# nianticlabs/mickey

Hardware: NVIDIA H100
Metric: image-pairs/sec @720x540 (higher is better)
Workload: dtype f16 operands / f32 accumulate (tensor core), f32 matcher+solver

## Files before the change

mickey_b200/csrc/attention_tc.cu:

```cuda
#include "gemm_tc.cuh"
#include "ops.h"
#include "gemm.h"
#include <algorithm>
#include <cstdlib>
#include <cstring>

namespace mk {

constexpr int FA_BQ = 192, FA_BK = 128, FA_D = 64, FA_KV_STAGES = 4;
constexpr int FA_CONSUMERS = 3, FA_THREADS = 128 * (FA_CONSUMERS + 1), FA_WARP_TMA = 4 * FA_CONSUMERS;
constexpr int FA_REGS_PRODUCER = 32, FA_REGS_CONSUMER = 160;
static_assert(FA_REGS_PRODUCER * 128 + FA_REGS_CONSUMER * 128 * FA_CONSUMERS <= 65536, "attention: register budget");
constexpr int FA_Q_BYTES = FA_BQ * 128;
constexpr int FA_KV_BYTES = FA_BK * 128;
constexpr int FA_O_BYTES = 64 * 128;
constexpr int FA_REGION = 2 * FA_Q_BYTES + 2 * FA_KV_STAGES * FA_KV_BYTES + FA_CONSUMERS * FA_O_BYTES;
constexpr int FA_SMEM = FA_REGION + 1024 + 256;
static_assert(FA_SMEM <= 227 * 1024, "attention: shared memory");

__device__ __forceinline__ float ex2_approx(float x) {
  float y;
  asm("ex2.approx.ftz.f32 %0, %1;" : "=f"(y) : "f"(x));
  return y;
}

__device__ __forceinline__ void wgmma_m64n64k16_rs_tb(float (&d)[32], const uint32_t (&a)[4], uint64_t desc_b) {
  asm volatile(
      "{\n\t.reg .pred p;\n\tsetp.ne.b32 p, %37, 0;\n\t"
      "wgmma.mma_async.sync.aligned.m64n64k16.f32.f16.f16 "
      "{%0, %1, %2, %3, %4, %5, %6, %7, %8, %9, %10, %11, %12, %13, %14, %15, %16, %17, %18, %19, %20, %21, %22, %23, %24, %25, %26, %27, %28, %29, %30, %31}, {%32, %33, %34, %35}, %36, p, 1, 1, 1;\n\t}"
      : "+f"(d[0]), "+f"(d[1]), "+f"(d[2]), "+f"(d[3]), "+f"(d[4]), "+f"(d[5]), "+f"(d[6]), "+f"(d[7]), "+f"(d[8]), "+f"(d[9]), "+f"(d[10]), "+f"(d[11]), "+f"(d[12]), "+f"(d[13]), "+f"(d[14]), "+f"(d[15]), "+f"(d[16]), "+f"(d[17]), "+f"(d[18]), "+f"(d[19]), "+f"(d[20]), "+f"(d[21]), "+f"(d[22]), "+f"(d[23]), "+f"(d[24]), "+f"(d[25]), "+f"(d[26]), "+f"(d[27]), "+f"(d[28]), "+f"(d[29]), "+f"(d[30]), "+f"(d[31])
      : "r"(a[0]), "r"(a[1]), "r"(a[2]), "r"(a[3]), "l"(desc_b), "r"(1u));
}

__device__ __forceinline__ void warpgroup_sync(int wg) { asm volatile("bar.sync %0, 128;" ::"r"(2 + wg) : "memory"); }

struct AttnTile { int qt, head, im; };
__device__ __forceinline__ AttnTile attn_tile(int t, int q_tiles, int heads) {
  const int bh = t / q_tiles;
  return {t - bh * q_tiles, bh % heads, bh / heads};
}

__device__ __forceinline__ void softmax_tile(float (&s)[64], uint32_t (&p)[8][4], float (&m_run)[2], float (&l_run)[2],
                                             float (&alpha)[2], float scale_log2, int valid, int lane) {
  if (valid < FA_BK) {
#pragma unroll
    for (int i = 0; i < 64; ++i) {
      const int col = 8 * (i >> 2) + 2 * (lane & 3) + (i & 1);
      if (col >= valid) s[i] = -INFINITY;
    }
  }
#pragma unroll
  for (int h = 0; h < 2; ++h) {
    float mx = -INFINITY;
#pragma unroll
    for (int c = 0; c < 16; ++c) mx = fmaxf(mx, fmaxf(s[4 * c + 2 * h], s[4 * c + 2 * h + 1]));
    mx = fmaxf(mx, __shfl_xor_sync(0xffffffffu, mx, 1));
    mx = fmaxf(mx, __shfl_xor_sync(0xffffffffu, mx, 2));
    const float m_new = fmaxf(m_run[h], mx * scale_log2);
    alpha[h] = ex2_approx(m_run[h] - m_new);
    m_run[h] = m_new;
    float sum = 0.f;
#pragma unroll
    for (int c = 0; c < 16; ++c) {
      const float p0 = ex2_approx(fmaf(s[4 * c + 2 * h], scale_log2, -m_new));
      const float p1 = ex2_approx(fmaf(s[4 * c + 2 * h + 1], scale_log2, -m_new));
      const __half2 ph = __floats2half2_rn(p0, p1);
      const float2 r = __half22float2(ph);
      p[c >> 1][2 * (c & 1) + h] = *reinterpret_cast<const uint32_t*>(&ph);
      sum += r.x + r.y;
    }
    l_run[h] = l_run[h] * alpha[h] + sum;
  }
}

__global__ void __launch_bounds__(FA_THREADS, 1)
attention_tc_kernel(const __grid_constant__ CUtensorMap tmQ, const __grid_constant__ CUtensorMap tmKV,
                    const __grid_constant__ CUtensorMap tmO, int T, int heads, int q_tiles, int n_tiles_total, float scale_log2) {
  extern __shared__ uint8_t smem_raw[];
  const uint32_t raw = smem_u32(smem_raw);
  const uint32_t base = (raw + 1023u) & ~1023u;
  const uint32_t sQ = base;
  const uint32_t sK = sQ + 2 * FA_Q_BYTES;
  const uint32_t sV = sK + FA_KV_STAGES * FA_KV_BYTES;
  const uint32_t sO = sV + FA_KV_STAGES * FA_KV_BYTES;
  const uint32_t bars = base + FA_REGION;
  const uint32_t k_full = bars, k_empty = k_full + 8 * FA_KV_STAGES, v_full = k_empty + 8 * FA_KV_STAGES,
                 v_empty = v_full + 8 * FA_KV_STAGES, q_full = v_empty + 8 * FA_KV_STAGES, q_empty = q_full + 16;

  const int warp = threadIdx.x >> 5, lane = threadIdx.x & 31;
  const int D = heads * FA_D;
  const int n_kv = (T + FA_BK - 1) / FA_BK;

  if (warp == FA_WARP_TMA && lane == 0) {
    asm volatile("prefetch.tensormap [%0];" ::"l"(&tmQ) : "memory");
    asm volatile("prefetch.tensormap [%0];" ::"l"(&tmKV) : "memory");
    asm volatile("prefetch.tensormap [%0];" ::"l"(&tmO) : "memory");
    for (int s = 0; s < FA_KV_STAGES; ++s) {
      mbar_init(k_full + 8 * s, 1); mbar_init(k_empty + 8 * s, 4 * FA_CONSUMERS);
      mbar_init(v_full + 8 * s, 1); mbar_init(v_empty + 8 * s, 4 * FA_CONSUMERS);
    }
    for (int b = 0; b < 2; ++b) { mbar_init(q_full + 8 * b, 1); mbar_init(q_empty + 8 * b, 4 * FA_CONSUMERS); }
    asm volatile("fence.mbarrier_init.release.cluster;" ::: "memory");
  }
  __syncthreads();
  pdl_wait();

  if (warp >= FA_WARP_TMA) {
    setmaxnreg_dec<FA_REGS_PRODUCER>();
    if (warp == FA_WARP_TMA && elect_one()) {
      int st = 0;
      uint32_t ph = 0;
      int it = 0;
      for (int t = blockIdx.x; t < n_tiles_total; t += gridDim.x, ++it) {
        const AttnTile tile = attn_tile(t, q_tiles, heads);
        const int row_base = tile.im * T;
        const int qb = it & 1;
        mbar_wait(q_empty + 8 * qb, ((it >> 1) & 1) ^ 1);
        mbar_expect_tx(q_full + 8 * qb, FA_Q_BYTES);
        tma_load_2d(sQ + qb * FA_Q_BYTES, &tmQ, q_full + 8 * qb, tile.head * FA_D, row_base + tile.qt * FA_BQ);
        for (int j = 0; j < n_kv; ++j) {
          mbar_wait(k_empty + 8 * st, ph ^ 1);
          mbar_expect_tx(k_full + 8 * st, FA_KV_BYTES);
          tma_load_2d(sK + st * FA_KV_BYTES, &tmKV, k_full + 8 * st, D + tile.head * FA_D, row_base + j * FA_BK);
          mbar_wait(v_empty + 8 * st, ph ^ 1);
          mbar_expect_tx(v_full + 8 * st, FA_KV_BYTES);
          tma_load_2d(sV + st * FA_KV_BYTES, &tmKV, v_full + 8 * st, 2 * D + tile.head * FA_D, row_base + j * FA_BK);
          if (++st == FA_KV_STAGES) { st = 0; ph ^= 1; }
        }
      }
    }
    __syncwarp();
    pdl_trigger();
    return;
  }

  setmaxnreg_inc<FA_REGS_CONSUMER>();
  const int wg = warp >> 2;
  const uint32_t stage_o = sO + wg * FA_O_BYTES;
  int ks = 0, vs = 0;
  uint32_t kph = 0, vph = 0;
  int it = 0;
  for (int t = blockIdx.x; t < n_tiles_total; t += gridDim.x, ++it) {
    const AttnTile tile = attn_tile(t, q_tiles, heads);
    const int qb = it & 1;
    const uint64_t dq = gmma_desc_sw128(sQ + qb * FA_Q_BYTES + wg * (64 * 128));
    float s[64], o[32];
    uint32_t p[8][4];
#pragma unroll
    for (int i = 0; i < 32; ++i) o[i] = 0.f;
    float m_run[2] = {-INFINITY, -INFINITY}, l_run[2] = {0.f, 0.f}, alpha[2];
    mbar_wait(q_full + 8 * qb, (it >> 1) & 1);

    for (int j = 0; j < n_kv; ++j) {
      mbar_wait(k_full + 8 * ks, kph);
      const uint64_t dk = gmma_desc_sw128(sK + ks * FA_KV_BYTES);
      wgmma_fence();
#pragma unroll
      for (int k = 0; k < FA_D / WGMMA_K; ++k) wgmma_m64n128k16(s, dq + (uint64_t)(k * 2), dk + (uint64_t)(k * 2), k > 0 ? 1u : 0u);
      wgmma_commit();
      wgmma_wait<0>();
      reg_fence(s);
      if (lane == 0) mbar_arrive(k_empty + 8 * ks);
      if (++ks == FA_KV_STAGES) { ks = 0; kph ^= 1; }
      softmax_tile(s, p, m_run, l_run, alpha, scale_log2, T - j * FA_BK, lane);
#pragma unroll
      for (int c = 0; c < 8; ++c) {
        o[4 * c] *= alpha[0]; o[4 * c + 1] *= alpha[0];
        o[4 * c + 2] *= alpha[1]; o[4 * c + 3] *= alpha[1];
      }
      mbar_wait(v_full + 8 * vs, vph);
      const uint64_t dv = gmma_desc_sw128(sV + vs * FA_KV_BYTES);
      wgmma_fence();
#pragma unroll
      for (int kk = 0; kk < FA_BK / WGMMA_K; ++kk)
        wgmma_m64n64k16_rs_tb(o, p[kk], dv + (uint64_t)(kk * 128));
      wgmma_commit();
      wgmma_wait<0>();
      reg_fence(o);
      if (lane == 0) mbar_arrive(v_empty + 8 * vs);
      if (++vs == FA_KV_STAGES) { vs = 0; vph ^= 1; }
    }
    if (lane == 0) mbar_arrive(q_empty + 8 * qb);
    if (t + (int)gridDim.x >= n_tiles_total) pdl_trigger();

    const int row0 = tile.qt * FA_BQ + wg * 64;
    if (row0 >= T) continue;
    if (threadIdx.x % 128 == 0) tma_store_wait_read();
    warpgroup_sync(wg);
#pragma unroll
    for (int h = 0; h < 2; ++h) {
      float l = l_run[h];
      l += __shfl_xor_sync(0xffffffffu, l, 1);
      l += __shfl_xor_sync(0xffffffffu, l, 2);
      const float inv = 1.0f / l;
      const int r = (warp & 3) * 16 + (lane >> 2) + 8 * h;
#pragma unroll
      for (int c = 0; c < 8; ++c) {
        const __half2 v = __floats2half2_rn(o[4 * c + 2 * h] * inv, o[4 * c + 2 * h + 1] * inv);
        asm volatile("st.shared.b32 [%0], %1;" ::"r"(stage_o + r * 128 + ((c ^ (r & 7)) << 4) + 4 * (lane & 3)),
                     "r"(*reinterpret_cast<const uint32_t*>(&v)) : "memory");
      }
    }
    fence_async_smem();
    warpgroup_sync(wg);
    if (threadIdx.x % 128 == 0) {
      tma_store_3d(&tmO, stage_o, tile.head * FA_D, row0, tile.im);
      tma_store_commit();
    }
  }
  if (threadIdx.x % 128 == 0) tma_store_wait_all();
}

int attention_tc(const void* qkv, void* out, int n_img, int T, int D, int heads, cudaStream_t s) {
  if (D != heads * FA_D) { set_last_error("attention: head_dim must be 64 (D=%d heads=%d)", D, heads); return MK_ERR_UNSUPPORTED; }
  static unsigned long long attr_mask = 0;
  if (first_use_on_device(attr_mask)) {
    MK_CUDA_CHECK(cudaFuncSetAttribute(attention_tc_kernel, cudaFuncAttributeMaxDynamicSharedMemorySize, FA_SMEM));
  }
  CUtensorMap tmQ, tmKV, tmO;
  int rc = make_tensor_map_f16(&tmQ, qkv, (long long)n_img * T, 3LL * D, 3LL * D, FA_BQ);
  if (!rc) rc = make_tensor_map_f16(&tmKV, qkv, (long long)n_img * T, 3LL * D, 3LL * D, FA_BK);
  if (!rc) rc = make_tensor_map_out_f16(&tmO, out, n_img, T, D, 64);
  if (rc) return rc;
  const int q_tiles = ceil_div(T, FA_BQ);
  const int tiles = q_tiles * heads * n_img;
  const float scale_log2 = 0.125f * 1.4426950408889634f;
  MK_CUDA_CHECK(launch_k(attention_tc_kernel, dim3(std::min(tiles, sm_count())), dim3(FA_THREADS), (size_t)FA_SMEM, s, tmQ, tmKV, tmO,
                         T, heads, q_tiles, tiles, scale_log2));
  return MK_OK;
}

int attention_dispatch(const void* qkv, void* out, int n_img, int T, int D, int heads, int impl, cudaStream_t s) {
  if (impl == 0) {
    static int def = 0;
    if (!def) { const char* e = getenv("MICKEY_ATTN_IMPL"); def = (e && strcmp(e, "mma") == 0) ? 2 : 1; }
    impl = def;
  }
  if (impl != 1 && impl != 2) { set_last_error("attention: unknown impl %d", impl); return MK_ERR_INVALID; }
  return impl == 2 ? attention(qkv, out, n_img, T, D, heads, s) : attention_tc(qkv, out, n_img, T, D, heads, s);
}

}
```

Measured before the change: 292.9.

## Pipeline QK and PV wgmma across iterations with ping-pong warpgroup scheduling

Splits the softmax into an exponent step and a pack step so that the next tile's QK wgmma and the current PV wgmma are issued together, overlapping tensor-core work with softmax math. Named barriers pass a turn between the consumer warpgroups so they alternate issuing MMAs, in the style of FA3 ping-pong. Masking becomes a compile-time template used only on the last KV block, and warpgroups whose 64-row slice lies fully past T now skip compute while still releasing pipeline slots. The q-tile order is also rotated per head. The pipelined variant is selected when T exceeds two KV blocks, at the cost of more registers and more complex barrier logic.

```diff
diff --git a/mickey_b200/csrc/attention_tc.cu b/mickey_b200/csrc/attention_tc.cu
--- a/mickey_b200/csrc/attention_tc.cu
+++ b/mickey_b200/csrc/attention_tc.cu
@@ -4,6 +4,7 @@
 #include <algorithm>
 #include <cstdlib>
 #include <cstring>
+#include <type_traits>
 
 namespace mk {
 
@@ -34,16 +35,22 @@
 }
 
 __device__ __forceinline__ void warpgroup_sync(int wg) { asm volatile("bar.sync %0, 128;" ::"r"(2 + wg) : "memory"); }
+constexpr int FA_BAR_TURN = 5;
+__device__ __forceinline__ void turn_wait(int wg) { asm volatile("bar.sync %0, 256;" ::"r"(FA_BAR_TURN + wg) : "memory"); }
+__device__ __forceinline__ void turn_pass(int wg) {
+  asm volatile("bar.arrive %0, 256;" ::"r"(FA_BAR_TURN + (wg + 1) % FA_CONSUMERS) : "memory");
+}
 
 struct AttnTile { int qt, head, im; };
 __device__ __forceinline__ AttnTile attn_tile(int t, int q_tiles, int heads) {
   const int bh = t / q_tiles;
-  return {t - bh * q_tiles, bh % heads, bh / heads};
-}
-
-__device__ __forceinline__ void softmax_tile(float (&s)[64], uint32_t (&p)[8][4], float (&m_run)[2], float (&l_run)[2],
-                                             float (&alpha)[2], float scale_log2, int valid, int lane) {
-  if (valid < FA_BK) {
+  return {(t - bh * q_tiles + bh) % q_tiles, bh % heads, bh / heads};
+}
+
+template <bool MASK>
+__device__ __forceinline__ void softmax_exp(float (&s)[64], float (&m_run)[2], float (&alpha)[2], float scale_log2,
+                                            int valid, int lane) {
+  if constexpr (MASK) {
 #pragma unroll
     for (int i = 0; i < 64; ++i) {
       const int col = 8 * (i >> 2) + 2 * (lane & 3) + (i & 1);
@@ -60,12 +67,22 @@
     const float m_new = fmaxf(m_run[h], mx * scale_log2);
     alpha[h] = ex2_approx(m_run[h] - m_new);
     m_run[h] = m_new;
+#pragma unroll
+    for (int c = 0; c < 16; ++c) {
+      s[4 * c + 2 * h] = ex2_approx(fmaf(s[4 * c + 2 * h], scale_log2, -m_new));
+      s[4 * c + 2 * h + 1] = ex2_approx(fmaf(s[4 * c + 2 * h + 1], scale_log2, -m_new));
+    }
+  }
+}
+
+__device__ __forceinline__ void softmax_pack(const float (&s)[64], uint32_t (&p)[8][4], float (&l_run)[2],
+                                             const float (&alpha)[2]) {
+#pragma unroll
+  for (int h = 0; h < 2; ++h) {
     float sum = 0.f;
 #pragma unroll
     for (int c = 0; c < 16; ++c) {
-      const float p0 = ex2_approx(fmaf(s[4 * c + 2 * h], scale_log2, -m_new));
-      const float p1 = ex2_approx(fmaf(s[4 * c + 2 * h + 1], scale_log2, -m_new));
-      const __half2 ph = __floats2half2_rn(p0, p1);
+      const __half2 ph = __floats2half2_rn(s[4 * c + 2 * h], s[4 * c + 2 * h + 1]);
       const float2 r = __half22float2(ph);
       p[c >> 1][2 * (c & 1) + h] = *reinterpret_cast<const uint32_t*>(&ph);
       sum += r.x + r.y;
@@ -74,6 +91,7 @@
   }
 }
 
+template <bool PIPELINED>
 __global__ void __launch_bounds__(FA_THREADS, 1)
 attention_tc_kernel(const __grid_constant__ CUtensorMap tmQ, const __grid_constant__ CUtensorMap tmKV,
                     const __grid_constant__ CUtensorMap tmO, int T, int heads, int q_tiles, int n_tiles_total, float scale_log2) {
@@ -136,10 +154,11 @@
   }
 
   setmaxnreg_inc<FA_REGS_CONSUMER>();
-  const int wg = warp >> 2;
+  const int wg = __shfl_sync(0xffffffffu, warp >> 2, 0);
   const uint32_t stage_o = sO + wg * FA_O_BYTES;
   int ks = 0, vs = 0;
   uint32_t kph = 0, vph = 0;
+  if (PIPELINED && wg == FA_CONSUMERS - 1) turn_pass(wg);
   int it = 0;
   for (int t = blockIdx.x; t < n_tiles_total; t += gridDim.x, ++it) {
     const AttnTile tile = attn_tile(t, q_tiles, heads);
@@ -150,36 +169,85 @@
 #pragma unroll
     for (int i = 0; i < 32; ++i) o[i] = 0.f;
     float m_run[2] = {-INFINITY, -INFINITY}, l_run[2] = {0.f, 0.f}, alpha[2];
-    mbar_wait(q_full + 8 * qb, (it >> 1) & 1);
-
-    for (int j = 0; j < n_kv; ++j) {
+    const int valid_last = T - (n_kv - 1) * FA_BK;
+
+    auto issue_qk = [&]() {
       mbar_wait(k_full + 8 * ks, kph);
       const uint64_t dk = gmma_desc_sw128(sK + ks * FA_KV_BYTES);
       wgmma_fence();
 #pragma unroll
       for (int k = 0; k < FA_D / WGMMA_K; ++k) wgmma_m64n128k16(s, dq + (uint64_t)(k * 2), dk + (uint64_t)(k * 2), k > 0 ? 1u : 0u);
       wgmma_commit();
-      wgmma_wait<0>();
-      reg_fence(s);
+    };
+    auto release_k = [&]() {
       if (lane == 0) mbar_arrive(k_empty + 8 * ks);
       if (++ks == FA_KV_STAGES) { ks = 0; kph ^= 1; }
-      softmax_tile(s, p, m_run, l_run, alpha, scale_log2, T - j * FA_BK, lane);
+    };
+    auto issue_pv = [&]() {
 #pragma unroll
       for (int c = 0; c < 8; ++c) {
         o[4 * c] *= alpha[0]; o[4 * c + 1] *= alpha[0];
         o[4 * c + 2] *= alpha[1]; o[4 * c + 3] *= alpha[1];
       }
-      mbar_wait(v_full + 8 * vs, vph);
       const uint64_t dv = gmma_desc_sw128(sV + vs * FA_KV_BYTES);
       wgmma_fence();
 #pragma unroll
       for (int kk = 0; kk < FA_BK / WGMMA_K; ++kk)
         wgmma_m64n64k16_rs_tb(o, p[kk], dv + (uint64_t)(kk * 128));
       wgmma_commit();
+    };
+    auto release_v = [&]() {
+      if (lane == 0) mbar_arrive(v_empty + 8 * vs);
+      if (++vs == FA_KV_STAGES) { vs = 0; vph ^= 1; }
+    };
+    auto retire_pv = [&]() {
       wgmma_wait<0>();
       reg_fence(o);
-      if (lane == 0) mbar_arrive(v_empty + 8 * vs);
-      if (++vs == FA_KV_STAGES) { vs = 0; vph ^= 1; }
+      reg_fence(s);
+      release_v();
+    };
+    auto qk_sync = [&]() { issue_qk(); wgmma_wait<0>(); reg_fence(s); release_k(); };
+    auto pv_sync = [&]() { mbar_wait(v_full + 8 * vs, vph); softmax_pack(s, p, l_run, alpha); issue_pv(); wgmma_wait<0>(); reg_fence(o); release_v(); };
+    auto kv_step = [&](auto first, auto mask) {
+      if constexpr (!decltype(first)::value) retire_pv();
+      mbar_wait(v_full + 8 * vs, vph);
+      softmax_pack(s, p, l_run, alpha);
+      turn_wait(wg);
+      issue_qk();
+      issue_pv();
+      turn_pass(wg);
+      wgmma_wait<1>();
+      reg_fence(s);
+      release_k();
+      softmax_exp<decltype(mask)::value>(s, m_run, alpha, scale_log2, valid_last, lane);
+      reg_fence(s);
+    };
+
+    if (tile.qt * FA_BQ + wg * 64 >= T) {
+      for (int j = 0; j < n_kv; ++j) {
+        if (PIPELINED && j > 0) { turn_wait(wg); turn_pass(wg); }
+        mbar_wait(k_full + 8 * ks, kph);
+        release_k();
+        mbar_wait(v_full + 8 * vs, vph);
+        release_v();
+      }
+    } else if constexpr (PIPELINED) {
+      mbar_wait(q_full + 8 * qb, (it >> 1) & 1);
+      qk_sync();
+      softmax_exp<false>(s, m_run, alpha, scale_log2, valid_last, lane);
+      kv_step(std::true_type{}, std::false_type{});
+      for (int j = 2; j < n_kv - 1; ++j) kv_step(std::false_type{}, std::false_type{});
+      kv_step(std::false_type{}, std::true_type{});
+      retire_pv();
+      pv_sync();
+    } else {
+      mbar_wait(q_full + 8 * qb, (it >> 1) & 1);
+      for (int j = 0; j < n_kv; ++j) {
+        qk_sync();
+        if (j == n_kv - 1) softmax_exp<true>(s, m_run, alpha, scale_log2, valid_last, lane);
+        else softmax_exp<false>(s, m_run, alpha, scale_log2, valid_last, lane);
+        pv_sync();
+      }
     }
     if (lane == 0) mbar_arrive(q_empty + 8 * qb);
     if (t + (int)gridDim.x >= n_tiles_total) pdl_trigger();
@@ -209,6 +277,7 @@
       tma_store_commit();
     }
   }
+  if (PIPELINED && wg == 0) turn_wait(wg);
   if (threadIdx.x % 128 == 0) tma_store_wait_all();
 }
 
@@ -216,7 +285,8 @@
   if (D != heads * FA_D) { set_last_error("attention: head_dim must be 64 (D=%d heads=%d)", D, heads); return MK_ERR_UNSUPPORTED; }
   static unsigned long long attr_mask = 0;
   if (first_use_on_device(attr_mask)) {
-    MK_CUDA_CHECK(cudaFuncSetAttribute(attention_tc_kernel, cudaFuncAttributeMaxDynamicSharedMemorySize, FA_SMEM));
+    MK_CUDA_CHECK(cudaFuncSetAttribute(attention_tc_kernel<true>, cudaFuncAttributeMaxDynamicSharedMemorySize, FA_SMEM));
+    MK_CUDA_CHECK(cudaFuncSetAttribute(attention_tc_kernel<false>, cudaFuncAttributeMaxDynamicSharedMemorySize, FA_SMEM));
   }
   CUtensorMap tmQ, tmKV, tmO;
   int rc = make_tensor_map_f16(&tmQ, qkv, (long long)n_img * T, 3LL * D, 3LL * D, FA_BQ);
@@ -226,7 +296,7 @@
   const int q_tiles = ceil_div(T, FA_BQ);
   const int tiles = q_tiles * heads * n_img;
   const float scale_log2 = 0.125f * 1.4426950408889634f;
-  MK_CUDA_CHECK(launch_k(attention_tc_kernel, dim3(std::min(tiles, sm_count())), dim3(FA_THREADS), (size_t)FA_SMEM, s, tmQ, tmKV, tmO,
+  MK_CUDA_CHECK(launch_k(T > 2 * FA_BK ? attention_tc_kernel<true> : attention_tc_kernel<false>, dim3(std::min(tiles, sm_count())), dim3(FA_THREADS), (size_t)FA_SMEM, s, tmQ, tmKV, tmO,
                          T, heads, q_tiles, tiles, scale_log2));
   return MK_OK;
 }
```

Result: faster. 298.0, median of 6 (+1.8%).
